# diver-j/melgan-multi

Hardware: NVIDIA H100
Metric: generator_fwd_audio_frames_per_sec (higher is better)
Workload: dtype f32 in/out; products as 3 split-bf16 wgmma passes with fp32 accumulation (fp32-equivalent, ~1e-5)

## Files before the change

### melgan_multi_b200/csrc/mg_api.cu

```cuda
#include <new>
#include <stdlib.h>
#include <string.h>

#include "mg_common.cuh"

namespace mg {


static int *status_ptr(void *workspace, int B, int T) {
    return reinterpret_cast<int *>(reinterpret_cast<float *>(workspace) + ws_offset(6, (size_t)B, (size_t)T));
}

static int run_generator(const float *mel, void *audio, const RunTable &batch, float *ws, cudaStream_t s,
                         cudaEvent_t *ev, const float *mel_host = nullptr, void *audio_host = nullptr,
                         int precision = MG_GEN_PRECISION_FP32, bool pcm16 = false) {
    int *st = status_ptr(ws, batch.items(), batch.stride);
    MG_CUDA_TRY(cudaMemsetAsync(st, 0, sizeof(int), s));
    return launch_generator_tc(mel, audio, batch, ws, st, s, ev, mel_host, audio_host, precision, pcm16);
}

int check_precision(const char *fn, int precision) {
    if (precision != MG_GEN_PRECISION_FP32 && precision != MG_GEN_PRECISION_BF16)
        return set_error(MG_ERR_INVALID_ARGUMENT, "%s: unknown precision %d (MG_GEN_PRECISION_FP32 = 0, MG_GEN_PRECISION_BF16 = 1)", fn,
                         precision);
// ... 475 lines not shown
    MG_CUDA_TRY(cudaMemcpy(&st, status_ptr(const_cast<void *>(workspace), B, T), sizeof(int), cudaMemcpyDeviceToHost));
    if (st) return set_error(MG_ERR_CUDA, "tensor-core pipeline wait timed out (role code %d)", st);
    return MG_OK;
}

int mg_gen_convt(const void *packed, int stage, const float *x, float *y, int B, int Lin, void *stream) {
    if (!packed || !x || !y || x == y || stage < 0 || stage > 3 || B < 1 || Lin < 1)
        return set_error(MG_ERR_INVALID_ARGUMENT, "mg_gen_convt: bad argument");
    return run_one_kernel("mg_gen_convt", (cudaStream_t)stream, [&](int *st) {
        return launch_convt_tc(x, y, stage, RunTable::uniform(B, Lin, (const float *)packed), st, (cudaStream_t)stream);
    });
}

int mg_gen_conv_pre(const void *packed, const float *mel, float *y, int B, int T, void *stream) {
    if (!packed || !mel || !y || B < 1 || T < 1) return set_error(MG_ERR_INVALID_ARGUMENT, "mg_gen_conv_pre: bad argument");
    return run_one_kernel("mg_gen_conv_pre", (cudaStream_t)stream, [&](int *st) {
        return launch_gen_pre_tc(mel, y, RunTable::uniform(B, T, (const float *)packed), st, (cudaStream_t)stream);
    });
}

int mg_gen_resblock_post(const void *packed, const float *x, float *audio, int B, int L, void *stream) {
    if (!packed || !x || !audio || B < 1 || L < 1) return set_error(MG_ERR_INVALID_ARGUMENT, "mg_gen_resblock_post: bad argument");
    return run_one_kernel("mg_gen_resblock_post", (cudaStream_t)stream, [&](int *st) {
        return launch_resblock_tc(x, audio, 4, RunTable::uniform(B, L, (const float *)packed), st, (cudaStream_t)stream);
    });
}

int mg_gen_resblock_trace(const void *packed, int stage, const float *x, float *y, int B, int L, long long *trace_host) {
    if (!packed || !x || !y || x == y || !trace_host || !*resblock_config_name(stage, 0) || B < 1 || L < 1)
        return set_error(MG_ERR_INVALID_ARGUMENT, "mg_gen_resblock_trace: bad argument");
    int *st = nullptr;
    long long *tr = nullptr;
    MG_CUDA_TRY(cudaMalloc(&st, sizeof(int)));
    MG_CUDA_TRY(cudaMalloc(&tr, 128 * sizeof(long long)));
    cudaMemset(st, 0, sizeof(int));
    cudaMemset(tr, 0, 128 * sizeof(long long));
    int rc = launch_resblock_tc(x, y, stage, RunTable::uniform(B, L, (const float *)packed), st, 0, tr);
    if (rc == MG_OK && cudaDeviceSynchronize() != cudaSuccess) rc = set_error(MG_ERR_CUDA, "mg_gen_resblock_trace: kernel failed");
    if (rc == MG_OK) cudaMemcpy(trace_host, tr, 128 * sizeof(long long), cudaMemcpyDeviceToHost);
    cudaFree(st);
    cudaFree(tr);
    return rc;
}

int mg_gen_resblock(const void *packed, int stage, const float *x, float *y, int B, int L, void *stream) {
    if (!packed || !x || !y || x == y || stage < 0 || stage > 3 || B < 1 || L < 1)
        return set_error(MG_ERR_INVALID_ARGUMENT, "mg_gen_resblock: bad argument");
    return run_one_kernel("mg_gen_resblock", (cudaStream_t)stream, [&](int *st) {
        return launch_resblock_tc(x, y, stage, RunTable::uniform(B, L, (const float *)packed), st, (cudaStream_t)stream);
    });
}

int mg_gen_resup(const void *packed, int stage, const float *x, float *y, int B, int L, void *stream) {
    if (!packed || !x || !y || x == y || stage < 0 || stage > 2 || B < 1 || L < 1)
        return set_error(MG_ERR_INVALID_ARGUMENT, "mg_gen_resup: bad argument");
    return run_one_kernel("mg_gen_resup", (cudaStream_t)stream, [&](int *st) {
        return launch_resblock_tc(x, y, 20 + stage, RunTable::uniform(B, L, (const float *)packed), st, (cudaStream_t)stream);
    });
}

int mg_gen_upres(const void *packed, int stage, const float *x, float *y, int B, int Lin, void *stream) {
    if (!packed || !x || !y || x == y || (stage != 2 && stage != 3) || B < 1 || Lin < 1)
        return set_error(MG_ERR_INVALID_ARGUMENT, "mg_gen_upres: bad argument");
    return run_one_kernel("mg_gen_upres", (cudaStream_t)stream, [&](int *st) {
        return launch_resblock_tc(x, y, 10 + stage, RunTable::uniform(B, 2 * Lin, (const float *)packed), st, (cudaStream_t)stream);
    });
}

int mg_gen_upres_post(const void *packed, const float *x, float *audio, int B, int Lin, void *stream) {
    if (!packed || !x || !audio || (const void *)x == (const void *)audio || B < 1 || Lin < 1)
        return set_error(MG_ERR_INVALID_ARGUMENT, "mg_gen_upres_post: bad argument");
    return run_one_kernel("mg_gen_upres_post", (cudaStream_t)stream, [&](int *st) {
        return launch_resblock_tc(x, audio, 14, RunTable::uniform(B, 2 * Lin, (const float *)packed), st, (cudaStream_t)stream);
    });
}

const char *mg_gen_resblock_config(int code) { return resblock_config_name(code, 0); }
size_t mg_gen_tc_weight_offset(int front, int layer, int co, int ci, int tap, int h) {
    if (h < 0 || h > 1 || co < 0 || ci < 0 || tap < 0) return (size_t)-1;
    if (front) {
        if (layer < 2 || layer > 3 || tap > 3) return (size_t)-1;
        const int C = stage_cout(layer);
        if (co >= C || ci >= 2 * C) return (size_t)-1;
        return tc_region_start() + tc_upf_offset(layer) + 2 * upf_weight_index(C, ci, co, tap, h);
    }
    if (layer < 0) return (size_t)-1;
    if (layer == 0) {
        if (co >= kPreCout || ci >= kMelBins || tap >= kPreK) return (size_t)-1;
        return tc_region_start() + tc_pre_offset() + 2 * conv_tc_weight_index(kMelBins, kPreK, kPreNG, co, ci, tap, h);
    }
    if (layer <= 4) {
        const int s = layer - 1;
        if (co >= stage_cout(s) || ci >= stage_cin(s) || tap >= stage_kup(s)) return (size_t)-1;
        return tc_region_start() + tc_up_offset(s) + 2 * up_weight_index(s, ci, co, tap, h);
    }
    if (layer > 28 || tap > 2) return (size_t)-1;
// ... 251 lines not shown
```

### melgan_multi_b200/csrc/mg_common.cuh

```cuda
#pragma once
#include <cuda_runtime.h>
#include <stdarg.h>
#include <stdint.h>
#include <stdio.h>

#include "../../include/melgan_b200.h"
#include "mg_layout.h"

namespace mg {

constexpr int kNumSMs = 132;

char *error_buffer();
int set_error(int code, const char *fmt, ...);

#define MG_CUDA_TRY(expr)                                                                     \
    do {                                                                                      \
        cudaError_t err__ = (expr);                                                           \
        if (err__ != cudaSuccess)                                                             \
            return ::mg::set_error(MG_ERR_CUDA, "%s failed: %s (%s:%d)", #expr,               \
                                   cudaGetErrorString(err__), __FILE__, __LINE__);            \
    } while (0)

__device__ __forceinline__ float lrelu(float x) { return fmaxf(x, x * kSlope); }
// ... 197 lines not shown
int mel_tables_build(int sr, int n_mels, float fmin, float fmax, int norm, MelTables *t);
int mel_frames(int L);
int launch_mel(const void *tables, const float *audio, float *mel, int B, int L, cudaStream_t s);
size_t mel_backward_workspace_bytes(int B, int L);
int launch_mel_backward(const void *tables, const float *audio, const float *grad_mel, float *grad_audio, int B, int L,
                        void *workspace, size_t workspace_bytes, cudaStream_t s);
size_t stft_tables_bytes(int n_fft);
int stft_tables_build(int n_fft, int win_length, void *tables_host);
int stft_frames(int n_fft, int hop, int L);
int stft_check(const char *fn, int n_res, const void *const *tables, const int *n_fft, const int *hop, int B, int L, int *T);
void stft_workspace(int n_res, const int *n_fft, int B, const int *T, size_t *fwd, size_t *bwd);
int launch_stft_loss_forward(int n_res, const void *const *tables, const int *n_fft, const int *hop, const float *x, const float *y,
                             int B, int L, const int *T, float *sc, float *mag, void *workspace, cudaStream_t s);
int launch_stft_loss_backward(int n_res, const void *const *tables, const int *n_fft, const int *hop, const float *x, const float *y,
                              int B, int L, const int *T, const float *grad_sc, const float *grad_mag, const void *fwd_workspace,
                              float *grad_x, void *workspace, cudaStream_t s);
int launch_msd_forward(const void *packed, const float *y, int Bt, int L, float *const *fmaps, int *status, cudaStream_t s);
int launch_convt_tc(const float *x, float *y, int stage, const RunTable &batch, int *status, cudaStream_t s,
                    int precision = MG_GEN_PRECISION_FP32);
const char *convt_config_name(int stage);
const char *gen_pre_config_name();
int launch_chain_kernel(int k, const float *x, float *y, const RunTable &t, int *status, cudaStream_t st,
                        int precision);
int launch_resblock_tc(const float *x, float *y, int stage, const RunTable &batch, int *status, cudaStream_t s,
                       long long *trace = nullptr, int precision = MG_GEN_PRECISION_FP32);
int launch_resblock_tc_pcm16(const float *x, int16_t *y, const RunTable &batch, int *status, cudaStream_t s, int precision);

}
```

### melgan_multi_b200/csrc/mg_gen_pipeline.cu

```cuda
#include <stdlib.h>

#include "mg_common.cuh"

namespace mg {

static thread_local int g_tail_override = -1;
void generator_tc_set_tail(int mask) { g_tail_override = mask; }
int generator_tc_tail() {
    static const int env_mask = [] {
        const char *e = getenv("MG_GEN_TAIL");
        if (!e) return 0;
        int m = 0;
        for (; *e; ++e) m |= (*e >= '1' && *e <= '3') ? 1 << (*e - '0') : 0;
        return m;
    }();
    return g_tail_override >= 0 ? (g_tail_override & 0b1110) : env_mask;
}
bool generator_tc_default_chain() { return generator_tc_tail() == 0 && generator_tc_fused_up() == 2; }
int generator_tc_fused_up() {
    static const int mask = [] {
        const char *e = getenv("MG_GEN_FUSE_UP");
        if (!e) return 2;
        int m = 0;
        for (; *e; ++e) m |= (*e == '2') ? 1 : (*e == '3') ? 2 : 0;
// ... 30 lines not shown
const char *generator_tc_kernel_name(int i) {
    ChainStep st[12];
    const int n = build_chain(st);
    return (i >= 0 && i < n) ? st[i].name : "";
}

const char *generator_tc_kernel_config(int i, int T) {
    ChainStep st[12];
    const int n = build_chain(st);
    if (i < 0 || i >= n || T < 1) return "";
    int len = T;
    for (int k = 0; k <= i; ++k) {
        if (st[k].kind == 1) len *= stage_stride(st[k].arg);
        else if (st[k].kind == 2) {
            const int a = st[k].arg;
            const int Lk = (a >= 12 && a <= 14) ? 2 * len : len;
            if (k == i) return resblock_config_name(a, Lk);
            len = a >= 20 ? Lk * stage_stride(a - 20 + 1) : Lk;
        }
    }
    return st[i].kind == 0 ? "conv_rows_tc_kernel<ConvCfg<80,512,7>>" : "convt_tc_kernel";
}

static int generator_tc_chain(const float *mel, void *audio, const RunTable &batch, float *a0,
                              float *const *a, float *u, int *status, cudaStream_t s, cudaEvent_t *ev, int precision,
                              bool pcm16) {
    ChainStep st[12];
    const int n = build_chain(st);
    int rc;
    float *big[3] = {a[1], a[2], u};
    auto other = [&](const float *x, const float *y) -> float * {
        for (float *b : big)
            if (b != x && b != y) return b;
        return nullptr;
    };
    const float *cur = mel;
    int len = 1;
    for (int i = 0; i < n; ++i) {
        if (ev) MG_CUDA_TRY(cudaEventRecord(ev[i], s));
        const ChainStep &k = st[i];
        if (k.kind == 0) {
            if ((rc = launch_gen_pre_tc(cur, a0, batch, status, s))) return rc;
            cur = a0;
        } else if (k.kind == 1) {
            float *out = cur != u ? u : other(cur, nullptr);
            if ((rc = launch_convt_tc(cur, out, k.arg, batch.scaled(len), status, s, precision))) return rc;
            cur = out;
            len *= stage_stride(k.arg);
        } else {
            if (k.arg < 0) return set_error(MG_ERR_INVALID_ARGUMENT, "generator pipeline: MG_GEN_FUSE_UP=2 cannot be combined with a tail-fused up3");
            const bool last = k.arg == 4 || k.arg == 14;
            const bool front = k.arg >= 12 && k.arg <= 14, tailf = k.arg >= 20;
            const int Lk = front ? 2 * len : len;
            if (last && pcm16) {
                if (k.arg != 14) return set_error(MG_ERR_INVALID_ARGUMENT, "generator pipeline: int16 audio needs the default chain");
                if ((rc = launch_resblock_tc_pcm16(cur, static_cast<int16_t *>(audio), batch.scaled(Lk), status, s, precision)))
                    return rc;
                continue;
            }
            float *out = last ? static_cast<float *>(audio) : (k.arg <= 2 && cur != a[k.arg]) ? a[k.arg] : other(cur, nullptr);
            if ((rc = launch_resblock_tc(cur, out, k.arg, batch.scaled(Lk), status, s, nullptr, precision))) return rc;
            cur = out;
            len = tailf ? Lk * stage_stride(k.arg - 20 + 1) : Lk;
        }
    }
    if (ev) MG_CUDA_TRY(cudaEventRecord(ev[n], s));
    return MG_OK;
}

constexpr int kMaxDevices = 64;
struct SliceStreams {
    static constexpr int kMax = 8;
    cudaStream_t st[kMax - 1] = {};
    cudaEvent_t fork = nullptr, join[kMax - 1] = {};
    bool ready = false;
    int init() {
        if (ready) return MG_OK;
        for (int i = 0; i < kMax - 1; ++i) {
            MG_CUDA_TRY(cudaStreamCreateWithFlags(&st[i], cudaStreamNonBlocking));
            MG_CUDA_TRY(cudaEventCreateWithFlags(&join[i], cudaEventDisableTiming));
        }
        MG_CUDA_TRY(cudaEventCreateWithFlags(&fork, cudaEventDisableTiming));
        ready = true;
        return MG_OK;
// ... 44 lines not shown
        MG_CUDA_TRY(cudaEventRecord(ss.fork, s));
    }
    int forked = 0;
    for (int k = 0; k < slices && rc == MG_OK; ++k) {
        const int b0 = cut[k], nb = cut[k + 1] - b0;
        const RunTable part = batch.slice(b0, cut[k + 1]);
        cudaStream_t q = k == 0 ? s : ss.st[k - 1];
        auto slice = [&]() -> int {
            if (k > 0) {
                MG_CUDA_TRY(cudaStreamWaitEvent(q, ss.fork, 0));
                forked = k;
            }
            for (int r = 0; mel_host && r < part.n; ++r) {
                const size_t off = (b0 + part.item0[r]) * mel_item, rows = (size_t)(part.item0[r + 1] - part.item0[r]) * kMelBins;
                float *dst = const_cast<float *>(mel) + off;
                if (part.len[r] == T)
                    MG_CUDA_TRY(cudaMemcpyAsync(dst, mel_host + off, rows * T * sizeof(float), cudaMemcpyHostToDevice, q));
                else
                    MG_CUDA_TRY(cudaMemcpy2DAsync(dst, T * sizeof(float), mel_host + off, T * sizeof(float), part.len[r] * sizeof(float),
                                                  rows, cudaMemcpyHostToDevice, q));
            }
            float *a[3] = {base[1] + b0 * per_item[1], base[2] + b0 * per_item[2], base[3] + b0 * per_item[3]};
            char *audio_b = static_cast<char *>(audio) + b0 * audio_item;
            int r = generator_tc_chain(mel + b0 * mel_item, audio_b, part, base[0] + b0 * per_item[0], a,
                                       base[5] + b0 * per_item[5], status, q, ev, precision, pcm16);
            if (r) return r;
            if (audio_host)
                MG_CUDA_TRY(cudaMemcpyAsync(static_cast<char *>(audio_host) + b0 * audio_item, audio_b, nb * audio_item,
                                            cudaMemcpyDeviceToHost, q));
            return MG_OK;
        };
        rc = slice();
    }
    for (int k = 1; k <= forked; ++k) {
        cudaError_t e = cudaEventRecord(ss.join[k - 1], ss.st[k - 1]);
        if (e == cudaSuccess) e = cudaStreamWaitEvent(s, ss.join[k - 1], 0);
        if (e != cudaSuccess && rc == MG_OK) rc = set_error(MG_ERR_CUDA, "launch_generator_tc: joining slice %d: %s", k, cudaGetErrorString(e));
    }
    return rc;
}

}
```

### melgan_multi_b200/csrc/mg_gen_stream.cu

```cuda
#include <algorithm>
#include <new>
#include <string.h>

#include "mg_common.cuh"
#include "mg_tc.cuh"

namespace mg {

namespace {

constexpr int kKernels = 8;
constexpr int kLookahead = 1542;
constexpr int kC[9] = {80, 512, 256, 256, 128, 128, 64, 64, 1};
constexpr int kScale[9] = {1, 1, 8, 8, 64, 64, 128, 128, 256};
constexpr int kReach[9] = {0, 3, 28, 44, 356, 372, 745, 761, 1542};
constexpr int kRatio[kKernels] = {1, 8, 1, 8, 1, 2, 1, 2};
constexpr int kTail[kKernels] = {6, 1, 32, 1, 32, 1, 32, 20};

long long floor_div(long long a, long long b) { return a >= 0 ? a / b : -((-a + b - 1) / b); }

long long exact_hi(int k, long long F) {
    long long v = 0;
    switch (k) {
        case 0: v = F - 3; break;
// ... 117 lines not shown
    off = align256(off + (size_t)S * L.out_item * sizeof(float));
    L.total = off;
    return L;
}

struct Plan {
    AsmTable asm_[kKernels + 1];
    long long asm_elems[kKernels + 1];
    int items[kKernels], lens[kKernels][MG_GEN_RAGGED_MAX_B], stride[kKernels];
    int voice[kKernels][MG_GEN_RAGGED_MAX_B];
    long long F[MG_GEN_RAGGED_MAX_B][9];
    unsigned char par[MG_GEN_RAGGED_MAX_B][kKernels];
    int bound[MG_GEN_RAGGED_MAX_B];
    long long bytes;
};

}

int launch_chain_kernel(int k, const float *x, float *y, const RunTable &t, int *status, cudaStream_t st,
                        int precision) {
    switch (k) {
        case 0: return launch_gen_pre_tc(x, y, t, status, st);
        case 1: return launch_convt_tc(x, y, 0, t, status, st, precision);
        case 2: return launch_resblock_tc(x, y, 0, t, status, st, nullptr, precision);
        case 3: return launch_convt_tc(x, y, 1, t, status, st, precision);
        case 4: return launch_resblock_tc(x, y, 1, t, status, st, nullptr, precision);
        case 5: return launch_convt_tc(x, y, 2, t, status, st, precision);
        case 6: return launch_resblock_tc(x, y, 2, t, status, st, nullptr, precision);
        case 7: return launch_resblock_tc(x, y, 14, t.scaled(2), status, st, nullptr, precision);
    }
    return set_error(MG_ERR_INVALID_ARGUMENT, "launch_chain_kernel: kernel %d", k);
}

}

using namespace mg;

struct mg_gen_stream {
    int S, P, precision;
    char *state;
    size_t state_bytes;
    StateLayout L;
    long long F[MG_GEN_RAGGED_MAX_B][9];
    unsigned char par[MG_GEN_RAGGED_MAX_B][kKernels];
    int voice[MG_GEN_RAGGED_MAX_B];
    bool status_written, dry;
    Plan plan;
};

namespace mg {
namespace {

// ... 275 lines not shown
```

### melgan_multi_b200/csrc/mg_res_tc.cu

```cuda
#include <stdlib.h>
#include <string.h>

#include "mg_common.cuh"
#include "mg_tc.cuh"

namespace mg {
using namespace tc;

template <int C_, int NRB_, int RPW_, int NCP_, int NSTAGE_, bool POST_ = false, bool UPF_ = false, int UPT_ = 0, int CS_ = 1>
struct RbCfg {
    static constexpr int C = C_, NRB = NRB_, RPW = RPW_, NCP = NCP_, NSTAGE = NSTAGE_, UPT = UPT_, CS = CS_;
    static constexpr bool POST = POST_;
    static constexpr bool UPF = UPF_;
    static constexpr bool ONEPASS = false;
    using Out = float;
    static constexpr int P = 64 * NRB;
    static constexpr int NWG = NRB / RPW * NCP;
    static constexpr int NCONS = 128 * NWG;
    static constexpr int NT = NCONS + 32;
    static constexpr int NCW = C / NCP;
    static constexpr int SLACK = 16;
    static constexpr int HALO = 16 + (POST ? 3 : 0);
    static constexpr int HL = HALO + (UPT_ ? 1 : 0);
    static constexpr int ROWS = P + 2 * SLACK;
    static constexpr int XPITCH = ROWS * 16;
    static constexpr int KP = C / 8;
    static constexpr int XBYTES = KP * XPITCH;
    static constexpr int KC = tc_kc(C);
    static constexpr int CHUNK = tc_chunk_bytes(C);
    static constexpr int HALF = CHUNK / 2;
    static constexpr int NCHUNK = tc_chunks_per_conv(C);
    static constexpr int KSL = C / KC;
    static constexpr int TNG = UPT == 8 ? 32 : C / 2, TN = (UPT ? UPT : 1) * TNG, TNCG = (C / 2) / TNG;
    static constexpr int TSLOT = UPT == 8 ? 16384 : 128 * UPT * TNG, TNSLOT = UPT ? TNCG * (C / 16) * (UPT == 8 ? 2 : 1) : 0;
    static_assert(UPT == 0 || ((UPT == 2 || UPT == 8) && TN == C && TSLOT <= CHUNK && !POST_ && !UPF_), "tail ConvT shape");
    static_assert(UPT != 8 || NCW == 128, "stride-8 tail: each column part stores four phases of a channel as one float4");
    static constexpr int UROWS = P / 2 + 2, UPITCH = UROWS * 16, NPB = NRB / 2, UKSL = 2 * C / KC, NUPCH = UPF ? 4 * UKSL : 0;
    static constexpr int SPITCH = P + 4;
    static_assert(!UPF || (NCP == 1 && NPB <= NWG && 2 * KP * UPITCH <= XBYTES && C * SPITCH * 4 <= 2 * XBYTES),
                  "fused ConvT must fit the X region");
    static_assert(!POST || (C == 32 && NCP == 1), "conv_post fusion is for the 32-channel stage");
    static constexpr int PVB = CS * P - HALO - HL, XCH = 9;
// ... 1 lines not shown
                  "clusters are for the plain ResBlock");
    static constexpr int CB_UPF = 6 * C, CB_UPT = CB_UPF + (UPF_ ? C : 0), CB_POST = CB_UPT + (UPT_ ? C / 2 : 0);
    static constexpr int NCONST = CB_POST + (POST_ ? 32 * 8 + 4 : 0);
    static_assert(CB_POST % 4 == 0 && NCONST % 2 == 0, "conv_post weights are read as float4, the mbarriers follow");
    static constexpr int SMEM_BYTES = 2 * XBYTES + NSTAGE * CHUNK + (2 * C + NCONST) * 4 + (2 * NSTAGE + (CS > 1 ? 2 : 0) + 1) * 8;
    static_assert(SMEM_BYTES + 1024 <= 227 * 1024, "shared memory budget");
    static_assert(XPITCH / 16 < 16384, "LBO field");
    static_assert(NRB % RPW == 0 && C % NCP == 0 && NCW % 32 == 0, "warpgroup split");
};

template <class Cfg>
struct Pcm16 : Cfg {
    using Out = int16_t;
    static_assert(Cfg::POST, "int16 output is the audio of a conv_post configuration");
};

template <int RPW, int R>
__device__ __forceinline__ void acc_fence2(float (&a)[RPW][R]) {
#pragma unroll
    for (int r = 0; r < RPW; ++r) acc_fence<R>(a[r]);
}

template <class Cfg>
__global__ void __launch_bounds__(Cfg::NT, 1)
resblock_tc_kernel(const float *__restrict__ x, float *__restrict__ y_, int stage, const __grid_constant__ RunTable clusters,
                   int *__restrict__ status, long long *__restrict__ trace) {
    constexpr int C = Cfg::C, P = Cfg::P, SLACK = Cfg::SLACK, HALO = Cfg::HALO, HL = Cfg::HL;
    constexpr int XPITCH = Cfg::XPITCH, XBYTES = Cfg::XBYTES, KC = Cfg::KC, CHUNK = Cfg::CHUNK, NSTAGE = Cfg::NSTAGE;
    constexpr int NCONS = Cfg::NCONS, NCP = Cfg::NCP, NCW = Cfg::NCW, RPW = Cfg::RPW, KSL = Cfg::KSL, NA = NCW / 2;
    constexpr int CS = Cfg::CS, XCH = Cfg::XCH;
    constexpr bool ONE = Cfg::ONEPASS;
    constexpr int NPASS = ONE ? 1 : 3;
    constexpr bool STK = tc_stacked(C), PAIR = STK && !ONE;
    constexpr uint32_t WLO = STK ? C * 16 : Cfg::HALF, WKP = STK ? 2 * C * 16 : C * 16;
    static_assert(!STK || NCP == 1, "stacked weights: one column part");
    constexpr uint32_t WBYTES = ONE && !STK ? Cfg::HALF : CHUNK;
    static_assert(!ONE || Cfg::UPT == 0, "the single-pass variant has no tail ConvT");
    typename Cfg::Out *__restrict__ y = reinterpret_cast<typename Cfg::Out *>(y_);
    static_assert(Cfg::POST || sizeof(typename Cfg::Out) == sizeof(float), "int16 output is for the conv_post epilogue only");
    extern __shared__ __align__(1024) uint8_t smem[];
    uint8_t *Xh = smem, *Xl = smem + XBYTES, *ring = smem + 2 * XBYTES;
    float *pend = reinterpret_cast<float *>(ring + NSTAGE * CHUNK);
    float *b1s = pend + C;
    float *cst = b1s + C;
    uint64_t *full = reinterpret_cast<uint64_t *>(cst + Cfg::NCONST);
    uint64_t *empty = full + NSTAGE;
    uint64_t *hfull = empty + NSTAGE, *hfree = hfull + 1;
    int *item_len = reinterpret_cast<int *>(empty + NSTAGE + (CS > 1 ? 2 : 0));

    const int tid = threadIdx.x, warp = tid >> 5, lane = tid & 31;
    const int crank = blockIdx.x % CS;
    const RunPos cp = clusters.find(blockIdx.x / CS);
    const int clus = cp.unit, Ls = clusters.stride;
    auto voice_blob = [&]() {
        int c = blockIdx.x / CS;
        asm volatile("" : "+r"(c));
        return clusters.blob_at(c);
    };
    auto item = [&]() { return *reinterpret_cast<volatile int *>(&item_len[0]); };
    auto len = [&]() { return *reinterpret_cast<volatile int *>(&item_len[1]); };
    const int oc = clus == 0 ? 0 : (CS * P - HALO) + (clus - 1) * Cfg::PVB - HL;
    const int o = oc + crank * P;
    const int p_lo = (clus == 0 || crank > 0) ? 0 : HL, p_hi = (crank < CS - 1 || oc + CS * P >= cp.len) ? P : P - HALO;
    const bool interior = (o >= 0 && o + P <= cp.len);
    const int l0 = 5 + 6 * stage;

    if (tid == 0) {
        item_len[0] = cp.item;
        item_len[1] = cp.len;
        for (int s = 0; s < NSTAGE; ++s) {
            mbar_init(&full[s], 1);
            mbar_init(&empty[s], Cfg::NWG * CS);
        }
        if constexpr (CS > 1) {
            mbar_init(hfull, 1);
            mbar_init(hfree, (crank > 0) + (crank < CS - 1));
        }
        fence_mbar_init();
    }
    for (int i = Cfg::UPF ? 1 << 30 : tid; i < 2 * Cfg::KP * 2 * SLACK; i += Cfg::NT) {
        const int r = i % (2 * SLACK), kp = (i / (2 * SLACK)) % Cfg::KP, hl = i / (2 * SLACK * Cfg::KP);
        const int row = r < SLACK ? r : P + r;
        *reinterpret_cast<uint4 *>((hl ? Xl : Xh) + kp * XPITCH + row * 16) = make_uint4(0, 0, 0, 0);
    }
    for (int i = tid; i < C; i += Cfg::NT) pend[i] = 0.f;
    const float *packed = voice_blob();
    for (int i = tid; i < Cfg::NCONST; i += Cfg::NT) {
        float v = 0.f;
        if (i < Cfg::CB_UPF) v = __ldg(packed + bias_offset(l0) + i);
        else if (i < Cfg::CB_UPT) v = __ldg(packed + bias_offset(1 + stage) + (i - Cfg::CB_UPF));
        else if (i < Cfg::CB_POST) v = __ldg(packed + bias_offset(1 + stage + 1) + (i - Cfg::CB_UPT));
        else if (i < Cfg::CB_POST + 32 * 8) {
            const int j = i - Cfg::CB_POST;
            if ((j & 7) < kPostK) v = __ldg(packed + weight_offset(29) + (j >> 3) * kPostK + (j & 7));
        } else if (i == Cfg::CB_POST + 32 * 8) {
            v = __ldg(packed + bias_offset(29));
        }
        cst[i] = v;
    }
    fence_proxy_async();
    __syncthreads();
    if constexpr (CS > 1) cluster_sync();
    const bool tr = trace && blockIdx.x == (gridDim.x > 1 ? 1u : 0u) && tid == 0;
#define MG_TR(slot) do { if (tr) trace[slot] = clock64(); } while (0)

    if (warp == NCONS / 32) {
        if (lane == 0) {
            const uint8_t *tc_base = reinterpret_cast<const uint8_t *>(voice_blob()) + tc_region_start();
            int s = 0, ph = 0, j = 0;
            bool ok = true;
            auto put = [&](const uint8_t *src, uint32_t bytes) {
                if (!ok || !mbar_wait(&empty[s], ph ^ 1)) { ok = false; return; }
                mbar_arrive_expect_tx(&full[s], bytes);
                if constexpr (CS == 1) bulk_g2s(ring + s * CHUNK, src, bytes, &full[s]);
                else if (j % CS == crank) bulk_g2s_multicast(ring + s * CHUNK, src, bytes, &full[s], (1 << CS) - 1);
                ++j;
                if (++s == NSTAGE) { s = 0; ph ^= 1; }
            };
            if constexpr (Cfg::UPF) {
                const uint8_t *src = tc_base + tc_upf_offset(stage);
                for (int i = 0; i < Cfg::NUPCH; ++i) put(src + (size_t)i * CHUNK, WBYTES);
            }
            for (int conv = 0; conv < 6; ++conv) {
                const uint8_t *src = tc_base + tc_res_offset(l0 + (conv >> 1) + 3 * (conv & 1));
                for (int i = 0; i < Cfg::NCHUNK; ++i) put(src + (size_t)i * CHUNK, WBYTES);
            }
            if constexpr (Cfg::UPT != 0) {
                const uint8_t *src = tc_base + tc_up_offset(stage + 1);
                for (int i = 0; i < Cfg::TNSLOT; ++i) put(src + (size_t)i * Cfg::TSLOT, Cfg::TSLOT);
            }
            if (!ok) atomicExch(status, 2);
        }
        if constexpr (CS > 1) cluster_sync();
        return;
    }

    const int wgi = warp >> 2, t = tid & 127, q = lane & 3;
    const int rb0 = (wgi / NCP) * RPW, c0 = (wgi % NCP) * NCW;
    const uint64_t adesc_t = desc_template(XPITCH, 128), bdesc_t = desc_template(WKP, 128);
    const uint32_t xh_addr = smem_u32(Xh), xl_addr = smem_u32(Xl), ring_addr = smem_u32(ring);
    float R[RPW][NA], D[RPW][NA];
    int s = 0, ph = 0, ps = -1;
    bool ok = true;
    auto release = [&](int slot) {
        if constexpr (CS == 1) {
            if (t == 0) mbar_arrive(&empty[slot]);
        } else if (t < CS) {
            mbar_arrive_remote(&empty[slot], t);
        }
    };
    auto chunk_begin = [&]() -> uint32_t {
        ok &= mbar_wait(&full[s], ph);
        acc_fence2(R);
        acc_fence2(D);
// ... 441 lines not shown
        for (int r = 0; r < RPW; ++r)
#pragma unroll
            for (int h = 0; h < 2; ++h) {
                const int p = (rb0 + r) * 64 + frag_row(t, h), tp = o + p;
                if (p >= p_lo && p < p_hi && tp < L) {
                    float *yp = y + (size_t)b * C * Ls + tp;
#pragma unroll
                    for (int k = 0; k < NCW / 8; ++k)
#pragma unroll
                        for (int e = 0; e < 2; ++e) {
                            const int col = c0 + frag_col(q, 4 * k + e);
                            yp[(size_t)col * Ls] = R[r][4 * k + 2 * h + e] + pend[col];
                        }
                }
            }
    }
    if (!ok && t == 0) atomicExch(status, 3);
    if constexpr (CS > 1) cluster_sync();
    MG_TR(20);
#undef MG_TR
}

template <class Cfg>
static int launch_resblock(const float *x, typename Cfg::Out *y, int stage, const RunTable &batch, int *status,
                           long long *trace, cudaStream_t s) {
    static bool configured = false;
    if (!configured) {
        MG_CUDA_TRY(cudaFuncSetAttribute(resblock_tc_kernel<Cfg>, cudaFuncAttributeMaxDynamicSharedMemorySize, Cfg::SMEM_BYTES));
        configured = true;
    }
    constexpr int CS = Cfg::CS, PC = CS * Cfg::P, PVB = Cfg::PVB;
    RunTable clusters = batch;
    clusters.set_units([](int L) { return 1 + (L > PC ? (L - PC + PVB - 1) / PVB : 0); });
    const dim3 grid(CS * clusters.first[clusters.n]);
    if (trace && CS > 1) {
        cudaLaunchConfig_t cfg{};
        cfg.gridDim = grid;
        cfg.blockDim = dim3(Cfg::NT);
        cfg.dynamicSmemBytes = Cfg::SMEM_BYTES;
        cudaLaunchAttribute attr;
        attr.id = cudaLaunchAttributeClusterDimension;
        attr.val.clusterDim.x = CS;
        attr.val.clusterDim.y = attr.val.clusterDim.z = 1;
        cfg.attrs = &attr;
        cfg.numAttrs = 1;
        int n = 0;
        MG_CUDA_TRY(cudaOccupancyMaxActiveClusters(&n, resblock_tc_kernel<Cfg>, &cfg));
        const long long v = n;
        MG_CUDA_TRY(cudaMemcpy(trace + 127, &v, sizeof(v), cudaMemcpyHostToDevice));
    }
    MG_CUDA_TRY(launch_ex(resblock_tc_kernel<Cfg>, grid, dim3(Cfg::NT), Cfg::SMEM_BYTES, s, true, CS, x, reinterpret_cast<float *>(y),
                          stage, clusters, status, trace));
    return MG_OK;
}

template <class Cfg>
static const char *cfg_name() {
    static char buf[96];
    snprintf(buf, sizeof(buf), "resblock_tc_kernel<RbCfg<%d,%d,%d,%d,%d,%d,%d,%d,%d>>", Cfg::C, Cfg::NRB, Cfg::RPW, Cfg::NCP,
             Cfg::NSTAGE, (int)Cfg::POST, (int)Cfg::UPF, Cfg::UPT, Cfg::CS);
    return buf;
}

using Rb0 = RbCfg<256, 1, 1, 2, 4, false, false, 0, 4>;
using Rb1 = RbCfg<128, 2, 1, 1, 4, false, false, 0, 2>;
using Rb2 = RbCfg<64, 4, 1, 1, 3>;
using Rb3 = RbCfg<32, 8, 2, 1, 4>;
using Rb3Post = RbCfg<32, 8, 2, 1, 4, true>;
using Up2Rb2 = RbCfg<64, 4, 1, 1, 3, false, true>;
using Up3Rb3 = RbCfg<32, 8, 2, 1, 4, false, true>;
using Up3Rb3Post = RbCfg<32, 8, 2, 1, 4, true, true>;
using Rb0Up1 = RbCfg<256, 1, 1, 2, 4, false, false, 8>;
using Rb1Up2 = RbCfg<128, 2, 1, 1, 4, false, false, 2>;
using Rb2Up3 = RbCfg<64, 4, 1, 1, 3, false, false, 2>;

int launch_resblock_tc(const float *x, float *y, int stage, const RunTable &batch, int *status, cudaStream_t s,
                       long long *trace, int precision) {
    if (precision == MG_GEN_PRECISION_BF16) {
        switch (stage) {
            case 0: return launch_resblock<Bf16<Rb0>>(x, y, 0, batch, status, trace, s);
            case 1: return launch_resblock<Bf16<Rb1>>(x, y, 1, batch, status, trace, s);
            case 2: return launch_resblock<Bf16<Rb2>>(x, y, 2, batch, status, trace, s);
            case 14: return launch_resblock<Bf16<Up3Rb3Post>>(x, y, 3, batch, status, trace, s);
        }
        return set_error(MG_ERR_INVALID_ARGUMENT, "launch_resblock_tc: stage code %d has no bf16 variant", stage);
    }
    if (precision != MG_GEN_PRECISION_FP32)
        return set_error(MG_ERR_INVALID_ARGUMENT, "launch_resblock_tc: precision %d", precision);
    switch (stage) {
        case 0: return launch_resblock<Rb0>(x, y, 0, batch, status, trace, s);
        case 1: return launch_resblock<Rb1>(x, y, 1, batch, status, trace, s);
        case 2: return launch_resblock<Rb2>(x, y, 2, batch, status, trace, s);
        case 3: return launch_resblock<Rb3>(x, y, 3, batch, status, trace, s);
        case 4: return launch_resblock<Rb3Post>(x, y, 3, batch, status, trace, s);
        case 12: return launch_resblock<Up2Rb2>(x, y, 2, batch, status, trace, s);
        case 13: return launch_resblock<Up3Rb3>(x, y, 3, batch, status, trace, s);
        case 14: return launch_resblock<Up3Rb3Post>(x, y, 3, batch, status, trace, s);
        case 20: return launch_resblock<Rb0Up1>(x, y, 0, batch, status, trace, s);
        case 21: return launch_resblock<Rb1Up2>(x, y, 1, batch, status, trace, s);
        case 22: return launch_resblock<Rb2Up3>(x, y, 2, batch, status, trace, s);
    }
    return set_error(MG_ERR_INVALID_ARGUMENT, "launch_resblock_tc: stage %d", stage);
}

int launch_resblock_tc_pcm16(const float *x, int16_t *y, const RunTable &batch, int *status, cudaStream_t s, int precision) {
    if (precision == MG_GEN_PRECISION_FP32) return launch_resblock<Pcm16<Up3Rb3Post>>(x, y, 3, batch, status, nullptr, s);
    if (precision == MG_GEN_PRECISION_BF16) return launch_resblock<Pcm16<Bf16<Up3Rb3Post>>>(x, y, 3, batch, status, nullptr, s);
    return set_error(MG_ERR_INVALID_ARGUMENT, "launch_resblock_tc_pcm16: precision %d", precision);
}

const char *resblock_config_name(int stage, int L) {
    (void)L;
    switch (stage) {
        case 0: return cfg_name<Rb0>();
        case 1: return cfg_name<Rb1>();
        case 2: return cfg_name<Rb2>();
        case 3: return cfg_name<Rb3>();
        case 4: return cfg_name<Rb3Post>();
        case 12: return cfg_name<Up2Rb2>();
        case 13: return cfg_name<Up3Rb3>();
        case 14: return cfg_name<Up3Rb3Post>();
        case 20: return cfg_name<Rb0Up1>();
        case 21: return cfg_name<Rb1Up2>();
        case 22: return cfg_name<Rb2Up3>();
    }
    return "";
}

}
```

### melgan_multi_b200/csrc/mg_tc.cuh

```cuda
#pragma once
#include <cuda_bf16.h>
#include <stdint.h>

namespace mg {
namespace tc {

__device__ __forceinline__ uint32_t smem_u32(const void *p) { return (uint32_t)__cvta_generic_to_shared(p); }

__device__ __forceinline__ void mbar_init(uint64_t *bar, uint32_t count) {
    asm volatile("mbarrier.init.shared::cta.b64 [%0], %1;" ::"r"(smem_u32(bar)), "r"(count));
}
__device__ __forceinline__ void fence_mbar_init() { asm volatile("fence.mbarrier_init.release.cluster;" ::: "memory"); }
__device__ __forceinline__ void mbar_arrive_expect_tx(uint64_t *bar, uint32_t bytes) {
    asm volatile("mbarrier.arrive.expect_tx.shared::cta.b64 _, [%0], %1;" ::"r"(smem_u32(bar)), "r"(bytes) : "memory");
}
__device__ __forceinline__ void mbar_arrive(uint64_t *bar) {
    asm volatile("mbarrier.arrive.shared::cta.b64 _, [%0];" ::"r"(smem_u32(bar)) : "memory");
}
__device__ __forceinline__ bool mbar_try_wait(uint64_t *bar, uint32_t parity) {
    uint32_t ok;
    asm volatile(
        "{\n\t.reg .pred p;\n\t"
        "mbarrier.try_wait.parity.shared::cta.b64 p, [%1], %2;\n\t"
        "selp.b32 %0, 1, 0, p;\n\t}"
// ... 13 lines not shown
    asm volatile("mapa.shared::cluster.u32 %0, %1, %2;" : "=r"(r) : "r"(addr), "r"(rank));
    return r;
}
__device__ __forceinline__ void mbar_arrive_remote(uint64_t *bar, uint32_t rank) {
    asm volatile("mbarrier.arrive.shared::cluster.b64 _, [%0];" ::"r"(mapa(smem_u32(bar), rank)) : "memory");
}
__device__ __forceinline__ void cluster_sync() {
    asm volatile("barrier.cluster.arrive.release;\n\tbarrier.cluster.wait.acquire;" ::: "memory");
}

__device__ __forceinline__ void bulk_g2s(void *smem_dst, const void *gmem_src, uint32_t bytes, uint64_t *bar) {
    asm volatile("cp.async.bulk.shared::cluster.global.mbarrier::complete_tx::bytes [%0], [%1], %2, [%3];" ::"r"(
                     smem_u32(smem_dst)),
                 "l"(gmem_src), "r"(bytes), "r"(smem_u32(bar))
                 : "memory");
}
__device__ __forceinline__ void bulk_g2s_multicast(void *smem_dst, const void *gmem_src, uint32_t bytes, uint64_t *bar,
                                                   uint16_t cta_mask) {
    asm volatile(
        "cp.async.bulk.shared::cluster.global.mbarrier::complete_tx::bytes.multicast::cluster [%0], [%1], %2, [%3], %4;" ::"r"(
            smem_u32(smem_dst)),
        "l"(gmem_src), "r"(bytes), "r"(smem_u32(bar)), "h"(cta_mask)
        : "memory");
}
__device__ __forceinline__ void bulk_s2s_cluster(uint32_t dst, uint32_t src, uint32_t bytes, uint32_t bar) {
    asm volatile("cp.async.bulk.shared::cluster.shared::cta.mbarrier::complete_tx::bytes [%0], [%1], %2, [%3];" ::"r"(dst), "r"(src),
                 "r"(bytes), "r"(bar)
                 : "memory");
}
__device__ __forceinline__ void fence_proxy_async() { asm volatile("fence.proxy.async.shared::cta;" ::: "memory"); }

__device__ __forceinline__ void named_bar_sync(int id, int count) {
    asm volatile("bar.sync %0, %1;" ::"r"(id), "r"(count) : "memory");
}

__device__ __forceinline__ void pdl_trigger() { asm volatile("griddepcontrol.launch_dependents;" ::: "memory"); }
__device__ __forceinline__ void pdl_wait() { asm volatile("griddepcontrol.wait;" ::: "memory"); }

__device__ __forceinline__ uint64_t desc_template(uint32_t lbo_bytes, uint32_t sbo_bytes) {
    return ((uint64_t)((lbo_bytes >> 4) & 0x3FFF) << 16) | ((uint64_t)((sbo_bytes >> 4) & 0x3FFF) << 32);
}
__device__ __forceinline__ uint64_t desc_at(uint64_t tmpl, uint32_t saddr) { return tmpl | (uint64_t)((saddr >> 4) & 0x3FFF); }

__device__ __forceinline__ void wgmma_fence() { asm volatile("wgmma.fence.sync.aligned;" ::: "memory"); }
__device__ __forceinline__ void wgmma_commit() { asm volatile("wgmma.commit_group.sync.aligned;" ::: "memory"); }
template <int N>
// ... 84 lines not shown
```

Measured before the change: 316.6 million.

## Add L2 prefetch warp in resblock kernel for the next wave's input tiles

Adds a second producer warp to the resblock kernel. Once the first pipeline stage is released, it issues cp.async.bulk.prefetch.L2 for the input rows of the block one resident wave ahead (pf blocks later). The prefetch distance is derived from an occupancy query that is cached per device and scaled by the number of concurrent chains. This aims to hide the global-memory latency of each block's initial activation load, at the cost of an extra 32 threads per block and extra L2 traffic.

```diff
diff --git a/melgan_multi_b200/csrc/mg_api.cu b/melgan_multi_b200/csrc/mg_api.cu
--- a/melgan_multi_b200/csrc/mg_api.cu
+++ b/melgan_multi_b200/csrc/mg_api.cu
@@ -521,7 +521,7 @@
 int mg_gen_resblock_post(const void *packed, const float *x, float *audio, int B, int L, void *stream) {
     if (!packed || !x || !audio || B < 1 || L < 1) return set_error(MG_ERR_INVALID_ARGUMENT, "mg_gen_resblock_post: bad argument");
     return run_one_kernel("mg_gen_resblock_post", (cudaStream_t)stream, [&](int *st) {
-        return launch_resblock_tc(x, audio, 4, RunTable::uniform(B, L, (const float *)packed), st, (cudaStream_t)stream);
+        return launch_resblock_tc(x, audio, 4, RunTable::uniform(B, L, (const float *)packed), 1, st, (cudaStream_t)stream);
     });
 }
 
@@ -534,7 +534,7 @@
     MG_CUDA_TRY(cudaMalloc(&tr, 128 * sizeof(long long)));
     cudaMemset(st, 0, sizeof(int));
     cudaMemset(tr, 0, 128 * sizeof(long long));
-    int rc = launch_resblock_tc(x, y, stage, RunTable::uniform(B, L, (const float *)packed), st, 0, tr);
+    int rc = launch_resblock_tc(x, y, stage, RunTable::uniform(B, L, (const float *)packed), 1, st, 0, tr);
     if (rc == MG_OK && cudaDeviceSynchronize() != cudaSuccess) rc = set_error(MG_ERR_CUDA, "mg_gen_resblock_trace: kernel failed");
     if (rc == MG_OK) cudaMemcpy(trace_host, tr, 128 * sizeof(long long), cudaMemcpyDeviceToHost);
     cudaFree(st);
@@ -546,7 +546,7 @@
     if (!packed || !x || !y || x == y || stage < 0 || stage > 3 || B < 1 || L < 1)
         return set_error(MG_ERR_INVALID_ARGUMENT, "mg_gen_resblock: bad argument");
     return run_one_kernel("mg_gen_resblock", (cudaStream_t)stream, [&](int *st) {
-        return launch_resblock_tc(x, y, stage, RunTable::uniform(B, L, (const float *)packed), st, (cudaStream_t)stream);
+        return launch_resblock_tc(x, y, stage, RunTable::uniform(B, L, (const float *)packed), 1, st, (cudaStream_t)stream);
     });
 }
 
@@ -554,7 +554,7 @@
     if (!packed || !x || !y || x == y || stage < 0 || stage > 2 || B < 1 || L < 1)
         return set_error(MG_ERR_INVALID_ARGUMENT, "mg_gen_resup: bad argument");
     return run_one_kernel("mg_gen_resup", (cudaStream_t)stream, [&](int *st) {
-        return launch_resblock_tc(x, y, 20 + stage, RunTable::uniform(B, L, (const float *)packed), st, (cudaStream_t)stream);
+        return launch_resblock_tc(x, y, 20 + stage, RunTable::uniform(B, L, (const float *)packed), 1, st, (cudaStream_t)stream);
     });
 }
 
@@ -562,7 +562,7 @@
     if (!packed || !x || !y || x == y || (stage != 2 && stage != 3) || B < 1 || Lin < 1)
         return set_error(MG_ERR_INVALID_ARGUMENT, "mg_gen_upres: bad argument");
     return run_one_kernel("mg_gen_upres", (cudaStream_t)stream, [&](int *st) {
-        return launch_resblock_tc(x, y, 10 + stage, RunTable::uniform(B, 2 * Lin, (const float *)packed), st, (cudaStream_t)stream);
+        return launch_resblock_tc(x, y, 10 + stage, RunTable::uniform(B, 2 * Lin, (const float *)packed), 1, st, (cudaStream_t)stream);
     });
 }
 
@@ -570,7 +570,7 @@
     if (!packed || !x || !audio || (const void *)x == (const void *)audio || B < 1 || Lin < 1)
         return set_error(MG_ERR_INVALID_ARGUMENT, "mg_gen_upres_post: bad argument");
     return run_one_kernel("mg_gen_upres_post", (cudaStream_t)stream, [&](int *st) {
-        return launch_resblock_tc(x, audio, 14, RunTable::uniform(B, 2 * Lin, (const float *)packed), st, (cudaStream_t)stream);
+        return launch_resblock_tc(x, audio, 14, RunTable::uniform(B, 2 * Lin, (const float *)packed), 1, st, (cudaStream_t)stream);
     });
 }
 
diff --git a/melgan_multi_b200/csrc/mg_common.cuh b/melgan_multi_b200/csrc/mg_common.cuh
--- a/melgan_multi_b200/csrc/mg_common.cuh
+++ b/melgan_multi_b200/csrc/mg_common.cuh
@@ -243,8 +243,9 @@
 const char *gen_pre_config_name();
 int launch_chain_kernel(int k, const float *x, float *y, const RunTable &t, int *status, cudaStream_t st,
                         int precision);
-int launch_resblock_tc(const float *x, float *y, int stage, const RunTable &batch, int *status, cudaStream_t s,
+int launch_resblock_tc(const float *x, float *y, int stage, const RunTable &batch, int chains, int *status, cudaStream_t s,
                        long long *trace = nullptr, int precision = MG_GEN_PRECISION_FP32);
-int launch_resblock_tc_pcm16(const float *x, int16_t *y, const RunTable &batch, int *status, cudaStream_t s, int precision);
-
-}
+int launch_resblock_tc_pcm16(const float *x, int16_t *y, const RunTable &batch, int chains, int *status, cudaStream_t s,
+                             int precision);
+
+}
diff --git a/melgan_multi_b200/csrc/mg_gen_pipeline.cu b/melgan_multi_b200/csrc/mg_gen_pipeline.cu
--- a/melgan_multi_b200/csrc/mg_gen_pipeline.cu
+++ b/melgan_multi_b200/csrc/mg_gen_pipeline.cu
@@ -76,7 +76,7 @@
     return st[i].kind == 0 ? "conv_rows_tc_kernel<ConvCfg<80,512,7>>" : "convt_tc_kernel";
 }
 
-static int generator_tc_chain(const float *mel, void *audio, const RunTable &batch, float *a0,
+static int generator_tc_chain(const float *mel, void *audio, const RunTable &batch, int chains, float *a0,
                               float *const *a, float *u, int *status, cudaStream_t s, cudaEvent_t *ev, int precision,
                               bool pcm16) {
     ChainStep st[12];
@@ -108,12 +108,12 @@
             const int Lk = front ? 2 * len : len;
             if (last && pcm16) {
                 if (k.arg != 14) return set_error(MG_ERR_INVALID_ARGUMENT, "generator pipeline: int16 audio needs the default chain");
-                if ((rc = launch_resblock_tc_pcm16(cur, static_cast<int16_t *>(audio), batch.scaled(Lk), status, s, precision)))
+                if ((rc = launch_resblock_tc_pcm16(cur, static_cast<int16_t *>(audio), batch.scaled(Lk), chains, status, s, precision)))
                     return rc;
                 continue;
             }
             float *out = last ? static_cast<float *>(audio) : (k.arg <= 2 && cur != a[k.arg]) ? a[k.arg] : other(cur, nullptr);
-            if ((rc = launch_resblock_tc(cur, out, k.arg, batch.scaled(Lk), status, s, nullptr, precision))) return rc;
+            if ((rc = launch_resblock_tc(cur, out, k.arg, batch.scaled(Lk), chains, status, s, nullptr, precision))) return rc;
             cur = out;
             len = tailf ? Lk * stage_stride(k.arg - 20 + 1) : Lk;
         }
@@ -204,7 +204,7 @@
             }
             float *a[3] = {base[1] + b0 * per_item[1], base[2] + b0 * per_item[2], base[3] + b0 * per_item[3]};
             char *audio_b = static_cast<char *>(audio) + b0 * audio_item;
-            int r = generator_tc_chain(mel + b0 * mel_item, audio_b, part, base[0] + b0 * per_item[0], a,
+            int r = generator_tc_chain(mel + b0 * mel_item, audio_b, part, slices, base[0] + b0 * per_item[0], a,
                                        base[5] + b0 * per_item[5], status, q, ev, precision, pcm16);
             if (r) return r;
             if (audio_host)
diff --git a/melgan_multi_b200/csrc/mg_gen_stream.cu b/melgan_multi_b200/csrc/mg_gen_stream.cu
--- a/melgan_multi_b200/csrc/mg_gen_stream.cu
+++ b/melgan_multi_b200/csrc/mg_gen_stream.cu
@@ -163,12 +163,12 @@
     switch (k) {
         case 0: return launch_gen_pre_tc(x, y, t, status, st);
         case 1: return launch_convt_tc(x, y, 0, t, status, st, precision);
-        case 2: return launch_resblock_tc(x, y, 0, t, status, st, nullptr, precision);
+        case 2: return launch_resblock_tc(x, y, 0, t, 1, status, st, nullptr, precision);
         case 3: return launch_convt_tc(x, y, 1, t, status, st, precision);
-        case 4: return launch_resblock_tc(x, y, 1, t, status, st, nullptr, precision);
+        case 4: return launch_resblock_tc(x, y, 1, t, 1, status, st, nullptr, precision);
         case 5: return launch_convt_tc(x, y, 2, t, status, st, precision);
-        case 6: return launch_resblock_tc(x, y, 2, t, status, st, nullptr, precision);
-        case 7: return launch_resblock_tc(x, y, 14, t.scaled(2), status, st, nullptr, precision);
+        case 6: return launch_resblock_tc(x, y, 2, t, 1, status, st, nullptr, precision);
+        case 7: return launch_resblock_tc(x, y, 14, t.scaled(2), 1, status, st, nullptr, precision);
     }
     return set_error(MG_ERR_INVALID_ARGUMENT, "launch_chain_kernel: kernel %d", k);
 }
diff --git a/melgan_multi_b200/csrc/mg_res_tc.cu b/melgan_multi_b200/csrc/mg_res_tc.cu
--- a/melgan_multi_b200/csrc/mg_res_tc.cu
+++ b/melgan_multi_b200/csrc/mg_res_tc.cu
@@ -17,7 +17,7 @@
     static constexpr int P = 64 * NRB;
     static constexpr int NWG = NRB / RPW * NCP;
     static constexpr int NCONS = 128 * NWG;
-    static constexpr int NT = NCONS + 32;
+    static constexpr int NT = NCONS + 64;
     static constexpr int NCW = C / NCP;
     static constexpr int SLACK = 16;
     static constexpr int HALO = 16 + (POST ? 3 : 0);
@@ -65,9 +65,14 @@
 }
 
 template <class Cfg>
+__device__ __forceinline__ int cluster_origin(int clus) {
+    return clus == 0 ? 0 : (Cfg::CS * Cfg::P - Cfg::HALO) + (clus - 1) * Cfg::PVB - Cfg::HL;
+}
+
+template <class Cfg>
 __global__ void __launch_bounds__(Cfg::NT, 1)
 resblock_tc_kernel(const float *__restrict__ x, float *__restrict__ y_, int stage, const __grid_constant__ RunTable clusters,
-                   int *__restrict__ status, long long *__restrict__ trace) {
+                   int *__restrict__ status, long long *__restrict__ trace, int pf) {
     constexpr int C = Cfg::C, P = Cfg::P, SLACK = Cfg::SLACK, HALO = Cfg::HALO, HL = Cfg::HL;
     constexpr int XPITCH = Cfg::XPITCH, XBYTES = Cfg::XBYTES, KC = Cfg::KC, CHUNK = Cfg::CHUNK, NSTAGE = Cfg::NSTAGE;
     constexpr int NCONS = Cfg::NCONS, NCP = Cfg::NCP, NCW = Cfg::NCW, RPW = Cfg::RPW, KSL = Cfg::KSL, NA = NCW / 2;
@@ -102,7 +107,7 @@
     };
     auto item = [&]() { return *reinterpret_cast<volatile int *>(&item_len[0]); };
     auto len = [&]() { return *reinterpret_cast<volatile int *>(&item_len[1]); };
-    const int oc = clus == 0 ? 0 : (CS * P - HALO) + (clus - 1) * Cfg::PVB - HL;
+    const int oc = cluster_origin<Cfg>(clus);
     const int o = oc + crank * P;
     const int p_lo = (clus == 0 || crank > 0) ? 0 : HL, p_hi = (crank < CS - 1 || oc + CS * P >= cp.len) ? P : P - HALO;
     const bool interior = (o >= 0 && o + P <= cp.len);
@@ -147,8 +152,8 @@
     const bool tr = trace && blockIdx.x == (gridDim.x > 1 ? 1u : 0u) && tid == 0;
 #define MG_TR(slot) do { if (tr) trace[slot] = clock64(); } while (0)
 
-    if (warp == NCONS / 32) {
-        if (lane == 0) {
+    if (warp >= NCONS / 32) {
+        if (warp == NCONS / 32 && lane == 0) {
             const uint8_t *tc_base = reinterpret_cast<const uint8_t *>(voice_blob()) + tc_region_start();
             int s = 0, ph = 0, j = 0;
             bool ok = true;
@@ -173,6 +178,22 @@
                 for (int i = 0; i < Cfg::TNSLOT; ++i) put(src + (size_t)i * Cfg::TSLOT, Cfg::TSLOT);
             }
             if (!ok) atomicExch(status, 2);
+        } else if (warp > NCONS / 32 && pf > 0) {
+            pdl_wait();
+            mbar_wait(&empty[0], 0, 1u << 20);
+            const unsigned nb = blockIdx.x + pf;
+            const RunPos np = nb < gridDim.x ? clusters.find(nb / CS) : RunPos{-1, 0, 0};
+            if (np.item >= 0) {
+                const int on = cluster_origin<Cfg>(np.unit) + crank * P;
+                constexpr int NCH = Cfg::UPF ? 2 * C : C;
+                const int xs = Cfg::UPF ? Ls >> 1 : Ls, xl = Cfg::UPF ? np.len >> 1 : np.len;
+                const int s0 = Cfg::UPF ? (on >> 1) - 1 : on, s1 = s0 + (Cfg::UPF ? Cfg::UROWS : P);
+                const int r0 = max(s0, 0) & ~3, r1 = (min(s1, xl) + 3) & ~3;
+                if (r0 < r1) {
+                    const float *base = x + (size_t)np.item * NCH * xs + r0;
+                    for (int c = lane; c < NCH; c += 32) bulk_prefetch_l2(base + (size_t)c * xs, (uint32_t)(r1 - r0) * 4);
+                }
+            }
         }
         if constexpr (CS > 1) cluster_sync();
         return;
@@ -660,8 +681,36 @@
 }
 
 template <class Cfg>
+static int resident_clusters(int *n) {
+    static thread_local int known[64] = {};
+    int dev = 0;
+    MG_CUDA_TRY(cudaGetDevice(&dev));
+    if (dev >= 0 && dev < 64 && known[dev] > 0) {
+        *n = known[dev];
+        return MG_OK;
+    }
+    if (Cfg::CS == 1) {
+        MG_CUDA_TRY(cudaDeviceGetAttribute(n, cudaDevAttrMultiProcessorCount, dev));
+    } else {
+        cudaLaunchConfig_t cfg{};
+        cfg.gridDim = dim3(Cfg::CS);
+        cfg.blockDim = dim3(Cfg::NT);
+        cfg.dynamicSmemBytes = Cfg::SMEM_BYTES;
+        cudaLaunchAttribute attr;
+        attr.id = cudaLaunchAttributeClusterDimension;
+        attr.val.clusterDim.x = Cfg::CS;
+        attr.val.clusterDim.y = attr.val.clusterDim.z = 1;
+        cfg.attrs = &attr;
+        cfg.numAttrs = 1;
+        MG_CUDA_TRY(cudaOccupancyMaxActiveClusters(n, resblock_tc_kernel<Cfg>, &cfg));
+    }
+    if (dev >= 0 && dev < 64) known[dev] = *n;
+    return MG_OK;
+}
+
+template <class Cfg>
 static int launch_resblock(const float *x, typename Cfg::Out *y, int stage, const RunTable &batch, int *status,
-                           long long *trace, cudaStream_t s) {
+                           long long *trace, int chains, cudaStream_t s) {
     static bool configured = false;
     if (!configured) {
         MG_CUDA_TRY(cudaFuncSetAttribute(resblock_tc_kernel<Cfg>, cudaFuncAttributeMaxDynamicSharedMemorySize, Cfg::SMEM_BYTES));
@@ -671,24 +720,17 @@
     RunTable clusters = batch;
     clusters.set_units([](int L) { return 1 + (L > PC ? (L - PC + PVB - 1) / PVB : 0); });
     const dim3 grid(CS * clusters.first[clusters.n]);
+    int resident = 0;
+    if (int rc = resident_clusters<Cfg>(&resident)) return rc;
+    const int xs = Cfg::UPF ? batch.stride / 2 : batch.stride;
+    const bool aligned = xs % 4 == 0 && reinterpret_cast<uintptr_t>(x) % 16 == 0;
+    const int pf = aligned ? resident / (chains > 2 ? chains / 2 : 1) * CS : 0;
     if (trace && CS > 1) {
-        cudaLaunchConfig_t cfg{};
-        cfg.gridDim = grid;
-        cfg.blockDim = dim3(Cfg::NT);
-        cfg.dynamicSmemBytes = Cfg::SMEM_BYTES;
-        cudaLaunchAttribute attr;
-        attr.id = cudaLaunchAttributeClusterDimension;
-        attr.val.clusterDim.x = CS;
-        attr.val.clusterDim.y = attr.val.clusterDim.z = 1;
-        cfg.attrs = &attr;
-        cfg.numAttrs = 1;
-        int n = 0;
-        MG_CUDA_TRY(cudaOccupancyMaxActiveClusters(&n, resblock_tc_kernel<Cfg>, &cfg));
-        const long long v = n;
+        const long long v = resident;
         MG_CUDA_TRY(cudaMemcpy(trace + 127, &v, sizeof(v), cudaMemcpyHostToDevice));
     }
     MG_CUDA_TRY(launch_ex(resblock_tc_kernel<Cfg>, grid, dim3(Cfg::NT), Cfg::SMEM_BYTES, s, true, CS, x, reinterpret_cast<float *>(y),
-                          stage, clusters, status, trace));
+                          stage, clusters, status, trace, pf));
     return MG_OK;
 }
 
@@ -712,38 +754,39 @@
 using Rb1Up2 = RbCfg<128, 2, 1, 1, 4, false, false, 2>;
 using Rb2Up3 = RbCfg<64, 4, 1, 1, 3, false, false, 2>;
 
-int launch_resblock_tc(const float *x, float *y, int stage, const RunTable &batch, int *status, cudaStream_t s,
+int launch_resblock_tc(const float *x, float *y, int stage, const RunTable &batch, int chains, int *status, cudaStream_t s,
                        long long *trace, int precision) {
     if (precision == MG_GEN_PRECISION_BF16) {
         switch (stage) {
-            case 0: return launch_resblock<Bf16<Rb0>>(x, y, 0, batch, status, trace, s);
-            case 1: return launch_resblock<Bf16<Rb1>>(x, y, 1, batch, status, trace, s);
-            case 2: return launch_resblock<Bf16<Rb2>>(x, y, 2, batch, status, trace, s);
-            case 14: return launch_resblock<Bf16<Up3Rb3Post>>(x, y, 3, batch, status, trace, s);
+            case 0: return launch_resblock<Bf16<Rb0>>(x, y, 0, batch, status, trace, chains, s);
+            case 1: return launch_resblock<Bf16<Rb1>>(x, y, 1, batch, status, trace, chains, s);
+            case 2: return launch_resblock<Bf16<Rb2>>(x, y, 2, batch, status, trace, chains, s);
+            case 14: return launch_resblock<Bf16<Up3Rb3Post>>(x, y, 3, batch, status, trace, chains, s);
         }
         return set_error(MG_ERR_INVALID_ARGUMENT, "launch_resblock_tc: stage code %d has no bf16 variant", stage);
     }
     if (precision != MG_GEN_PRECISION_FP32)
         return set_error(MG_ERR_INVALID_ARGUMENT, "launch_resblock_tc: precision %d", precision);
     switch (stage) {
-        case 0: return launch_resblock<Rb0>(x, y, 0, batch, status, trace, s);
-        case 1: return launch_resblock<Rb1>(x, y, 1, batch, status, trace, s);
-        case 2: return launch_resblock<Rb2>(x, y, 2, batch, status, trace, s);
-        case 3: return launch_resblock<Rb3>(x, y, 3, batch, status, trace, s);
-        case 4: return launch_resblock<Rb3Post>(x, y, 3, batch, status, trace, s);
-        case 12: return launch_resblock<Up2Rb2>(x, y, 2, batch, status, trace, s);
-        case 13: return launch_resblock<Up3Rb3>(x, y, 3, batch, status, trace, s);
-        case 14: return launch_resblock<Up3Rb3Post>(x, y, 3, batch, status, trace, s);
-        case 20: return launch_resblock<Rb0Up1>(x, y, 0, batch, status, trace, s);
-        case 21: return launch_resblock<Rb1Up2>(x, y, 1, batch, status, trace, s);
-        case 22: return launch_resblock<Rb2Up3>(x, y, 2, batch, status, trace, s);
+        case 0: return launch_resblock<Rb0>(x, y, 0, batch, status, trace, chains, s);
+        case 1: return launch_resblock<Rb1>(x, y, 1, batch, status, trace, chains, s);
+        case 2: return launch_resblock<Rb2>(x, y, 2, batch, status, trace, chains, s);
+        case 3: return launch_resblock<Rb3>(x, y, 3, batch, status, trace, chains, s);
+        case 4: return launch_resblock<Rb3Post>(x, y, 3, batch, status, trace, chains, s);
+        case 12: return launch_resblock<Up2Rb2>(x, y, 2, batch, status, trace, chains, s);
+        case 13: return launch_resblock<Up3Rb3>(x, y, 3, batch, status, trace, chains, s);
+        case 14: return launch_resblock<Up3Rb3Post>(x, y, 3, batch, status, trace, chains, s);
+        case 20: return launch_resblock<Rb0Up1>(x, y, 0, batch, status, trace, chains, s);
+        case 21: return launch_resblock<Rb1Up2>(x, y, 1, batch, status, trace, chains, s);
+        case 22: return launch_resblock<Rb2Up3>(x, y, 2, batch, status, trace, chains, s);
     }
     return set_error(MG_ERR_INVALID_ARGUMENT, "launch_resblock_tc: stage %d", stage);
 }
 
-int launch_resblock_tc_pcm16(const float *x, int16_t *y, const RunTable &batch, int *status, cudaStream_t s, int precision) {
-    if (precision == MG_GEN_PRECISION_FP32) return launch_resblock<Pcm16<Up3Rb3Post>>(x, y, 3, batch, status, nullptr, s);
-    if (precision == MG_GEN_PRECISION_BF16) return launch_resblock<Pcm16<Bf16<Up3Rb3Post>>>(x, y, 3, batch, status, nullptr, s);
+int launch_resblock_tc_pcm16(const float *x, int16_t *y, const RunTable &batch, int chains, int *status, cudaStream_t s,
+                             int precision) {
+    if (precision == MG_GEN_PRECISION_FP32) return launch_resblock<Pcm16<Up3Rb3Post>>(x, y, 3, batch, status, nullptr, chains, s);
+    if (precision == MG_GEN_PRECISION_BF16) return launch_resblock<Pcm16<Bf16<Up3Rb3Post>>>(x, y, 3, batch, status, nullptr, chains, s);
     return set_error(MG_ERR_INVALID_ARGUMENT, "launch_resblock_tc_pcm16: precision %d", precision);
 }
 
diff --git a/melgan_multi_b200/csrc/mg_tc.cuh b/melgan_multi_b200/csrc/mg_tc.cuh
--- a/melgan_multi_b200/csrc/mg_tc.cuh
+++ b/melgan_multi_b200/csrc/mg_tc.cuh
@@ -59,6 +59,9 @@
             smem_u32(smem_dst)),
         "l"(gmem_src), "r"(bytes), "r"(smem_u32(bar)), "h"(cta_mask)
         : "memory");
+}
+__device__ __forceinline__ void bulk_prefetch_l2(const void *gmem_src, uint32_t bytes) {
+    asm volatile("cp.async.bulk.prefetch.L2.global [%0], %1;" ::"l"(gmem_src), "r"(bytes) : "memory");
 }
 __device__ __forceinline__ void bulk_s2s_cluster(uint32_t dst, uint32_t src, uint32_t bytes, uint32_t bar) {
     asm volatile("cp.async.bulk.shared::cluster.shared::cta.mbarrier::complete_tx::bytes [%0], [%1], %2, [%3];" ::"r"(dst), "r"(src),
```

After: 317.7 million (median of 6 runs). Within noise of the previous version (+0.4%).
